# constantinpape/torch-em

Measured on AMD Instinct MI355X. Metric: voxels/sec fwd+bwd, UNet3d 1x128^3 bs=2, higher is better.
Workload: dtype f32-class (forward convs on normalised activations: fp32 operands split into 2 fp16 terms = 22 mantissa bits, lo plane scaled by 2^12 with its own fp32 accumulator, 3 fp16 MFMAs per product; other forward convs 3 bf16 terms / 6 MFMAs; data-gradient convs 2 bf16 terms / 3 MFMAs (16-bit products); WEI

## Files before the change

torch_em_amd/csrc/capi.hip:

```cpp
#include "tem_common.h"
#include "conv_internal.h"
#include "tem_act.h"
#include <stdarg.h>
#include <string.h>

static thread_local char g_err[512] = "";

thread_local TemCallSt tem_call_st = {0, 0};
thread_local TemCallCs tem_call_cs = {0, 0};

void tem_set_error(const char* fmt, ...) {
    va_list ap;
    va_start(ap, fmt);
    vsnprintf(g_err, sizeof(g_err), fmt, ap);
    va_end(ap);
}

extern "C" const char* tem_last_error(void) { return g_err; }

struct TemOption {
    const char* name;
    long long def;
};
static const TemOption g_opt_table[TEM_OPT_COUNT] = {
    {"wgrad_zs", 3},
    {"wgrad_zs_persist", 1},
    {"wgrad_sums", 1},
    {"wgrad_sums_min_mb", 128},
    {"fwd_persistent", -1},
    {"conv_fwd_variant", -1},
    {"conv1x1_stream", 1},
    {"fwd_ksplit_chunks", 0},
    {"wgrad_cus", 256},
    {"upsample_generic", 0},
    {"team_min_units", 0},
    {"zr_splitk", 1},
    {"zr_wide", 1},
    {"zr_tile_blocks", 1},
    {"dice_vox", 1},
    {"upsample2_ch8", 1},
    {"pool_vec8", 2},
    {"fp32_zr", 1},
};
static long long g_opt_val[TEM_OPT_COUNT];
static bool g_opt_set[TEM_OPT_COUNT];

long long tem_option(int id) {
    if (id < 0 || id >= TEM_OPT_COUNT) return 0;
    return __atomic_load_n(&g_opt_set[id], __ATOMIC_RELAXED) ? __atomic_load_n(&g_opt_val[id], __ATOMIC_RELAXED)
                                                            : g_opt_table[id].def;
}
static int opt_find(const char* name) {
    if (!name) return -1;
    for (int i = 0; i < TEM_OPT_COUNT; ++i)
        if (!strcmp(name, g_opt_table[i].name)) return i;
    return -1;
}
extern "C" int tem_set_option(const char* name, int64_t value) {
    const int id = opt_find(name);
    TEM_REQUIRE(id >= 0, "tem_set_option: unknown option '%s'", name ? name : "(null)");
    __atomic_store_n(&g_opt_val[id], (long long)value, __ATOMIC_RELAXED);
    __atomic_store_n(&g_opt_set[id], true, __ATOMIC_RELAXED);
    return TEM_OK;
}
extern "C" int tem_get_option(const char* name, int64_t* value) {
    const int id = opt_find(name);
    TEM_REQUIRE(id >= 0 && value, "tem_get_option: unknown option '%s'", name ? name : "(null)");
    *value = (int64_t)tem_option(id);
    return TEM_OK;
}
extern "C" int tem_version(void) { return 100; }

thread_local TemByproducts* tem_call_bp = nullptr;
unsigned* tem_take_output_amax() {
    TemByproducts* bp = tem_call_bp;
    if (!bp || !bp->out_amax || (bp->delivered & TEM_BP_OUT_AMAX)) return nullptr;
    bp->delivered |= TEM_BP_OUT_AMAX;
    return bp->out_amax;
}
bool tem_bp_wants(unsigned bit) {
    const TemByproducts* bp = tem_call_bp;
    if (!bp || (bp->delivered & bit)) return false;
    return bit == TEM_BP_NORM_COEF ? bp->coef != nullptr : bit == TEM_BP_NORM_SUMS ? bp->sums_part != nullptr : bp->out_amax != nullptr;
}
void tem_bp_delivered(unsigned bit) {
    if (tem_call_bp) tem_call_bp->delivered |= bit;
}

extern "C" int tem_device_cus(void) {
    int dev = 0;
    if (hipGetDevice(&dev) != hipSuccess) return TEM_ELAUNCH;
    hipDeviceProp_t prop;
    if (hipGetDeviceProperties(&prop, dev) != hipSuccess) return TEM_ELAUNCH;
    return prop.multiProcessorCount;
}
// ... 157 lines not shown
```

torch_em_amd/csrc/conv_zr.hip:

```cpp
#include "tem_common.h"
#include "conv_internal.h"
#include "conv_split.h"
#include "tem_act.h"
#include <type_traits>

#ifndef TEM_ZR_PRIO
#define TEM_ZR_PRIO 1
#endif
#ifndef TEM_ZR_STAGE_PRIO
#define TEM_ZR_STAGE_PRIO 0
#endif
#ifndef TEM_ZR_R0
#define TEM_ZR_R0 2
#endif
#ifndef TEM_ZR_R0_16
#define TEM_ZR_R0_16 2
#endif
#ifndef TEM_ZR_R0_16S
#define TEM_ZR_R0_16S 2
#endif
#ifndef TEM_ZR_AD
#define TEM_ZR_AD 2
#endif
#ifndef TEM_ZR_ST_AUX
#define TEM_ZR_ST_AUX 2
#endif
#ifndef TEM_ZR_ST_AUX_KS
#define TEM_ZR_ST_AUX_KS 2
#endif
#ifndef TEM_ZR_X32_SCHED
#define TEM_ZR_X32_SCHED 1
#endif
#ifndef TEM_ZR_X32_R0_M0
#define TEM_ZR_X32_R0_M0 6
#define TEM_ZR_X32_R0_M1 4
#define TEM_ZR_X32_R0_M2 6
#define TEM_ZR_X32_R0_M3 5
#endif
#ifndef TEM_ZR_X32_GAP
#define TEM_ZR_X32_GAP 0
#endif
#ifndef TEM_ZR_ABL
#define TEM_ZR_ABL 0
#endif

typedef float floatx4z __attribute__((ext_vector_type(4)));
typedef float float2v __attribute__((ext_vector_type(2)));
typedef unsigned int u32x4z __attribute__((ext_vector_type(4)));

__device__ __forceinline__ __amdgpu_buffer_rsrc_t zr_rsrc(const void* base) {
    return __builtin_amdgcn_make_buffer_rsrc(const_cast<void*>(base), 0, 0x7fffffff, 0x00020000);
}
__device__ __forceinline__ float4 zr_load4(__amdgpu_buffer_rsrc_t r, unsigned voff, unsigned soff) {
    const u32x4z v = __builtin_amdgcn_raw_buffer_load_b128(r, voff, soff, 0);
    const floatx4z f = __builtin_bit_cast(floatx4z, v);
    return make_float4(f.x, f.y, f.z, f.w);
}
__device__ __forceinline__ uint4 zr_load4u(__amdgpu_buffer_rsrc_t r, unsigned voff, unsigned soff) {
    const u32x4z v = __builtin_amdgcn_raw_buffer_load_b128(r, voff, soff, 0);
    return make_uint4(v.x, v.y, v.z, v.w);
}
template <int AUX>
__device__ __forceinline__ void zr_store4(__amdgpu_buffer_rsrc_t r, unsigned voff, unsigned soff, float a, float b, float c, float d) {
    const u32x4z v = {__builtin_bit_cast(unsigned, a), __builtin_bit_cast(unsigned, b), __builtin_bit_cast(unsigned, c),
                      __builtin_bit_cast(unsigned, d)};
    __builtin_amdgcn_raw_buffer_store_b128(v, r, voff + soff, 0, AUX);
}

__device__ __forceinline__ uint2 zr_load2u(__amdgpu_buffer_rsrc_t r, unsigned voff, unsigned soff) {
    typedef unsigned int u32x2z __attribute__((ext_vector_type(2)));
    const u32x2z v = __builtin_amdgcn_raw_buffer_load_b64(r, voff, soff, 0);
    return make_uint2(v.x, v.y);
}
template <int AUX>
__device__ __forceinline__ void zr_store2u(__amdgpu_buffer_rsrc_t r, unsigned voff, unsigned soff, unsigned a, unsigned b) {
    typedef unsigned int u32x2z __attribute__((ext_vector_type(2)));
    const u32x2z v = {a, b};
    __builtin_amdgcn_raw_buffer_store_b64(v, r, voff + soff, 0, AUX);
}
template <bool F16>
__device__ __forceinline__ unsigned zr_norm2(unsigned h, float s0, float t0, float s1, float t1) {
    if constexpr (F16) {
        unsigned q;
        asm("v_fma_mixlo_f16 %0, %1, %2, %3 op_sel_hi:[1,0,0]" : "=v"(q) : "v"(h), "v"(s0), "v"(t0));
        asm("v_fma_mixhi_f16 %0, %1, %2, %3 op_sel:[1,0,0] op_sel_hi:[1,0,0]" : "+v"(q) : "v"(h), "v"(s1), "v"(t1));
        return q;
    } else {
        const float a = __builtin_bit_cast(float, h << 16), b = __builtin_bit_cast(float, h & 0xffff0000u);
        return pk_bf16(fmaf(a, s0, t0), fmaf(b, s1, t1));
    }
}

template <int M>
__device__ __forceinline__ float zr_swz(float v) {
    return __builtin_bit_cast(float, __builtin_amdgcn_ds_swizzle(__builtin_bit_cast(int, v), (M << 10) | 0x1f));
}

__device__ __forceinline__ float zr_xor16_sum(float r) {
    float a = r, b = r;
    asm volatile("s_nop 1\n\tv_permlane16_swap_b32 %0, %1" : "+v"(a), "+v"(b));
    return a + b;
}
__device__ __forceinline__ float zr_xor32_sum(float r) {
    float a = r, b = r;
    asm volatile("s_nop 1\n\tv_permlane32_swap_b32 %0, %1" : "+v"(a), "+v"(b));
    return a + b;
}

template <int CTRL>
__device__ __forceinline__ float zr_dpp(float v) {
    return __builtin_bit_cast(float, __builtin_amdgcn_update_dpp(0, __builtin_bit_cast(int, v), CTRL, 0xf, 0xf, true));
}

__device__ __forceinline__ unsigned zr_mix_lo(unsigned h, float g0, float g1) {
    unsigned q;
    const float c = -F16_LO_SCALE;
    asm("v_fma_mixlo_f16 %0, %1, %2, %3 op_sel_hi:[1,0,0]" : "=v"(q) : "v"(h), "s"(c), "v"(g0));
    asm("v_fma_mixhi_f16 %0, %1, %2, %3 op_sel:[1,0,0] op_sel_hi:[1,0,0]" : "+v"(q) : "v"(h), "s"(c), "v"(g1));
    return q;
}

#ifdef TEM_ZR_TRACE
#ifndef TEM_ZR_TRACE_BLOCK
#define TEM_ZR_TRACE_BLOCK 0
#endif
__device__ unsigned long long tem_zr_trace_buf[2][64][12];
#define ZR_STAMP(i)                                                                           \
    do {                                                                                      \
        if (blockIdx.x == TEM_ZR_TRACE_BLOCK && tw == 0 && lane == 0 && s < 64)               \
            tem_zr_trace_buf[team][s][i] = __builtin_amdgcn_s_memtime();                      \
    } while (0)
void tem_zr_trace_read(unsigned long long* dst) {
    (void)hipMemcpyFromSymbol(dst, HIP_SYMBOL(tem_zr_trace_buf), sizeof(unsigned long long) * 2 * 64 * 12);
}
#else
#define ZR_STAMP(i) asm volatile("; ZRMARK " #i)
#endif

__device__ __forceinline__ void zr_x32_gap() {
    if constexpr (TEM_ZR_X32_GAP > 0) {
        __builtin_amdgcn_sched_barrier(0);
        constexpr int FULL16 = TEM_ZR_X32_GAP / 16, REST = TEM_ZR_X32_GAP % 16;
#pragma unroll
        for (int i = 0; i < FULL16; ++i) asm volatile("s_nop 15");
        if constexpr (REST > 0) asm volatile("s_nop %0" ::"n"(REST - 1));
        __builtin_amdgcn_sched_barrier(0);
    }
}

__device__ __forceinline__ unsigned zr_ssel_ltu(unsigned a, unsigned b, unsigned t, unsigned f) {
    unsigned r;
    asm volatile("s_cmp_lt_u32 %1, %2\n\ts_cselect_b32 %0, %3, %4" : "=s"(r) : "s"(a), "s"(b), "s"(t), "s"(f) : "scc");
    return r;
}

struct ZrUnit {
    int cot, n, z0, y0, x0, ksl;
};

template <int NS, bool F16, int MODE, bool KSPLIT = false, bool WIDE = false, typename T = float, bool X32 = false, bool XS = false>
__global__ __launch_bounds__(XS ? 256 : 512, XS ? 1 : 2) void k_conv_zr(
    const T* __restrict__ x, int64_t x_ld, const float* __restrict__ scale, const float* __restrict__ shift,
    const uint4* __restrict__ wp, const float* __restrict__ bias, std::conditional_t<KSPLIT, float, T>* __restrict__ y, int64_t y_ld,
    const T* __restrict__ ref, int64_t ref_ld, int N, int D, int H, int W, int Cin, int Cout, int act, int nZ,
    int nY, int nX, float* __restrict__ stat, int nunits, const unsigned* __restrict__ in_amax, int ks, int blk,
    unsigned* __restrict__ out_amax, int64_t x_cs, int64_t y_cs) {
    static_assert(!KSPLIT || MODE == 0, "split-K units write raw partial sums");
    constexpr bool AMAX = MODE == 2 || MODE == 3;
    float amx = 0.f;
    static_assert(!WIDE || NS == 2, "the wide one-term kernel uses the two LDS planes of the two-term layout");
    static_assert(!X32 || (NS == 2 && !F16 && !WIDE && sizeof(T) == 4), "exact fp32: two LDS planes of eight fp32 channels, fp32 tensors");
    static_assert(!XS || X32, "the one-team workgroup exists for the exact-fp32 arithmetic only");
    constexpr bool T16 = sizeof(T) == 2;
    using TOut = std::conditional_t<KSPLIT, float, T>;
    constexpr bool Y16 = sizeof(TOut) == 2;
    constexpr int XB = (int)sizeof(T), YB = (int)sizeof(TOut);
    static_assert(!T16 || WIDE, "16-bit storage: 32 input channels per phase");
    constexpr int CK = WIDE ? 2 * BCK : BCK;
    constexpr int TZ = 4, TY = 16, TX = 8;
    constexpr int HZ = TZ + 2, HY = TY + 2, HX = TX + 2;
    constexpr int HV = HZ * HY * HX;
    constexpr int PLB = HV * 32;
    constexpr int NIT = HZ * 3;
    constexpr int LPV = (WIDE && !T16) ? 8 : 4;
    constexpr int SPP = (WIDE && !T16) ? 6 : 3;
    constexpr int CPL = T16 ? 8 : 4;
    constexpr int RP = NIT / SPP;
    constexpr int R0 = X32 ? (MODE == 0 ? TEM_ZR_X32_R0_M0 : MODE == 1 ? TEM_ZR_X32_R0_M1 : MODE == 2 ? TEM_ZR_X32_R0_M2 : TEM_ZR_X32_R0_M3)
                       : (WIDE && !T16) ? ((MODE == 1 || MODE == 3) ? 1 : 2)
                       : T16 ? ((MODE == 1 || MODE == 3) ? TEM_ZR_R0_16S : TEM_ZR_R0_16)
                             : (TEM_ZR_R0 < HZ ? TEM_ZR_R0 : HZ);
    constexpr int FR = NS * 64;
    constexpr bool SC = F16 && NS == 2 && !WIDE;
    constexpr int ZSTEP = HY * HX * 32;
    static_assert(HY % 2 == 0, "the record-half swizzle (row parity) is the same in every halo plane");
    extern __shared__ __attribute__((aligned(16))) unsigned char zr_lds[];

    if (SC) __builtin_amdgcn_s_setreg(1 | (23 << 6) | (0 << 11), 1);
    const int tid = threadIdx.x, lane = tid & 63;
    const int wv = __builtin_amdgcn_readfirstlane(tid >> 6);
    const int team = wv >> 2, tw = wv & 3, tl = tid & 255;
    const int kh = lane >> 5, v = lane & 31;
    const int vu = (int)((0x73261540u >> (4 * (v >> 2))) & 7u) * 4 + (v & 3);
    const int py = vu >> 3, px = vu & 7;
    unsigned char* lds = zr_lds + team * (NS * PLB);

    const int G = (XS ? 1 : 2) * gridDim.x;
    const int slot = XS ? tem_xcd_remap(blockIdx.x, gridDim.x) : tem_xcd_remap(blockIdx.x, gridDim.x) * 2 + team;
    const int ncot = Cout >> 5;
    const int nch_all = Cin / CK;
    const int nch = KSPLIT ? nch_all / ks : nch_all;
    const int my_units = slot < nunits ? (nunits - slot + G - 1) / G : 0;
    const int P = ((nunits + G - 1) / G) * nch;

    auto decode = [&](int ui) {
        int u = slot + ui * G;
        ZrUnit t;
        t.ksl = 0;
        if (KSPLIT) { t.ksl = u % ks; u /= ks; }
// ... 198 lines not shown
                if ((u & 1) == 0) col_addr(u >> 1);
#pragma unroll
                for (int hz = 0; hz < HZ; ++hz) xr[u & 1][hz] = *reinterpret_cast<const uint4*>(tcur + a0 + hz * ZSTEP + (u & 1) * PLB);
            };
            r_read(0);
#pragma unroll
            for (int u = 0; u < 18; ++u) {
                const int g = u >> 1, p = u & 1;
                if (u + PFD < NSL) stage_load(u + PFD);
                if (u + 1 < 18) r_read(u + 1);
                if (g + 1 < 9 && !(TEM_ZR_ABL & 4)) {
                    const int gn = g + 1;
#pragma unroll
                    for (int tz = (p ? 2 : 0); tz < (p ? 3 : 2); ++tz)
#pragma unroll
                        for (int pp = 0; pp < 2; ++pp)
                            wq[gn & 1][tz][pp] = zr_load4u(rw, woff_lane, wsoff + (unsigned)((tz * 9 + gn) * ts + pp * 64) * 16u);
                }
                if (u >= 15) {
                    const int tz = u - 15;
#pragma unroll
                    for (int pp = 0; pp < 2; ++pp) wqn[tz][pp] = zr_load4u(rw, woff_lane, wsoff_n + (unsigned)((tz * 9) * ts + pp * 64) * 16u);
                }
                stage_conv(u, tnxt);
#pragma unroll
                for (int c = 0; c < 4; ++c)
#pragma unroll
                    for (int tz = 0; tz < 3; ++tz)
#pragma unroll
                        for (int z = 0; z < TZ; ++z)
                            acc[z] = __builtin_amdgcn_mfma_f32_32x32x2f32(comp(wq[g & 1][tz][p], c), comp(xr[u & 1][z + tz], c), acc[z], 0, 0, 0);
                __builtin_amdgcn_sched_barrier(0);
            }
            if (last_chunk) {
                eu = cu;
                bve = bv;
                unsigned yo = yoff_lane, ro = roff_lane;
                asm volatile("" : "+v"(yo), "+v"(ro));
                epilogue_now(yo, ro, ph);
                bv = bias ? bias[tu.cot * 32 + v] : 0.f;
                ++ui;
            }
            cu = tu;
            ci = tc;
#pragma unroll
            for (int tz = 0; tz < 3; ++tz)
#pragma unroll
                for (int p = 0; p < 2; ++p) wq[0][tz][p] = wqn[tz][p];
            __syncthreads();
        }
        if (AMAX && out_amax) tem_amax_commit(out_amax, amx);
        return;
    }
    if (team) __syncthreads();
    for (int s = 0; s <= P; ++s) {
        const bool do_stage = ui < my_units;
        uint4 wq[2][3][NS];
        {
            ZR_STAMP(0);
            if (TEM_ZR_STAGE_PRIO) __builtin_amdgcn_s_setprio(TEM_ZR_STAGE_PRIO);
#pragma unroll
            for (int j = 0; j < SPP; ++j) asm volatile("" : "+v"(lwj[j]), "+v"(poff[j]));
            unsigned yoff_l = yoff_lane, roff_l = roff_lane;
            asm volatile("" : "+v"(yoff_l), "+v"(roff_l));
            float4 tmp[NIT];
            unsigned inb[2] = {0xffffffffu, 0xffffffffu};
            float4 sc4 = make_float4(1.f, 1.f, 1.f, 1.f), sf4 = make_float4(0.f, 0.f, 0.f, 0.f);
            float4 sc5 = sc4, sf5 = sf4;
            bool interior = true;
            __amdgpu_buffer_rsrc_t rx = zr_rsrc(x);
            auto load_norm = [&]() {
                if (scale) {
                    sc4 = *reinterpret_cast<const float4*>(scale + (int64_t)cu.n * Cin + (cu.ksl * nch + ci) * CK + c4 * CPL);
                    sf4 = *reinterpret_cast<const float4*>(shift + (int64_t)cu.n * Cin + (cu.ksl * nch + ci) * CK + c4 * CPL);
                    if (T16) {
                        sc5 = *reinterpret_cast<const float4*>(scale + (int64_t)cu.n * Cin + (cu.ksl * nch + ci) * CK + c4 * CPL + 4);
                        sf5 = *reinterpret_cast<const float4*>(shift + (int64_t)cu.n * Cin + (cu.ksl * nch + ci) * CK + c4 * CPL + 4);
                    }
                } else if (in_amax) {
                    sc4 = make_float4(psc, psc, psc, psc);
                }
            };
            if (do_stage) {
                if constexpr (!X32) load_norm();
                const int64_t xch = (T16 && x_cs) ? (int64_t)(cu.ksl * nch + ci) * x_cs : (int64_t)((cu.ksl * nch + ci) * CK);
                const T* xb = x + ((((int64_t)cu.n * D + (cu.z0 - 1)) * H + (cu.y0 - 1)) * W + (cu.x0 - 1)) * x_ld + xch;
                rx = zr_rsrc((TEM_ZR_ABL & 64) ? x + xch : xb);
                interior = (cu.z0 >= 1) & (cu.z0 + HZ - 1 <= D) & (cu.y0 >= 1) & (cu.y0 + HY - 1 <= H) & (cu.x0 >= 1) &
                           (cu.x0 + HX - 1 <= W);
                if (TEM_ZR_ABL & 32) interior = true;
                if constexpr (X32) {
#pragma unroll
                    for (int hz = 0; hz < R0; ++hz) {
                        const unsigned so = zr_ssel_ltu((unsigned)(cu.z0 - 1 + hz), (unsigned)D, (unsigned)hz * plane_b, plane_b);
#pragma unroll
                        for (int j = 0; j < SPP; ++j) {
                            if (TEM_ZR_ABL & 1) tmp[hz * SPP + j] = make_float4(0.5f + hz, 0.25f, -1.f, 2.f);
                            else tmp[hz * SPP + j] = zr_load4(rx, pvo[X32 ? j : 0], so);
                        }
                    }
                    load_norm();
                }
            }
            unsigned yx = (1u << SPP) - 1u;
            if constexpr (X32) {
                if (do_stage) {
                    yx = yxu;
                    if (!interior) {
                        inb[0] = inb[1] = 0;
#pragma unroll
                        for (int hz = 0; hz < HZ; ++hz) {
                            const bool zok = (unsigned)(cu.z0 - 1 + hz) < (unsigned)D;
#pragma unroll
                            for (int j = 0; j < SPP; ++j)
                                inb[hz / 3] |= (zok & ((yx >> j) & 1u)) ? (1u << ((hz % 3) * SPP + j)) : 0u;
                        }
                    }
                }
            } else
            if (do_stage && !interior) {
                int tl_ = tl;
                asm volatile("" : "+v"(tl_));
                yx = 0;
#pragma unroll
                for (int j = 0; j < SPP; ++j) {
                    const int q = min((tl_ + 256 * j) / LPV, HY * HX - 1);
                    const unsigned gy = (unsigned)(cu.y0 - 1 + q / HX), gx = (unsigned)(cu.x0 - 1 + q % HX);
                    yx |= ((gy < (unsigned)H) & (gx < (unsigned)W)) ? (1u << j) : 0u;
                }
            }
            auto issue_loads = [&](auto interior_tag, auto lo_tag, auto hi_tag) {
                constexpr bool INTERIOR = decltype(interior_tag)::value;
                constexpr int LO = decltype(lo_tag)::value, HI = decltype(hi_tag)::value;
                if (INTERIOR) {
#pragma unroll
                    for (int hz = LO; hz < HI; ++hz)
#pragma unroll
                        for (int j = 0; j < SPP; ++j) {
                            if (TEM_ZR_ABL & 1) tmp[(hz % RP) * SPP + j] = make_float4(0.5f + hz, 0.25f, -1.f, 2.f);
                            else tmp[(hz % RP) * SPP + j] = zr_load4(rx, poff[j], (unsigned)hz * plane_b);
                        }
                } else {
                    if (LO == 0) inb[0] = inb[1] = 0;
#pragma unroll
                    for (int hz = LO; hz < HI; ++hz) {
                        const bool zok = (unsigned)(cu.z0 - 1 + hz) < (unsigned)D;
#pragma unroll
                        for (int j = 0; j < SPP; ++j) {
                            const bool ok = zok & ((yx >> j) & 1u);
                            inb[hz / 3] |= ok ? (1u << ((hz % 3) * SPP + j)) : 0u;
                            tmp[(hz % RP) * SPP + j] = zr_load4(rx, (ok ? poff[j] : ctr_off) + (ok ? (unsigned)hz * plane_b : plane_b), 0);
                        }
                    }
                }
            };
            if (do_stage && !X32) {
                if (interior) issue_loads(std::true_type{}, std::integral_constant<int, 0>{}, std::integral_constant<int, R0>{});
                else issue_loads(std::false_type{}, std::integral_constant<int, 0>{}, std::integral_constant<int, R0>{});
            }
            ZR_STAMP(1);
            if (!X32 && epi_pending) {
#include "conv_zr_epilogue.inc"
                epi_pending = false;
                ZR_STAMP(11);
            }
            ZR_STAMP(6);
            if (do_stage) {
                auto convert = [&](auto interior_tag, auto hz_tag) {
                    constexpr bool INTERIOR = decltype(interior_tag)::value;
                    constexpr int hz = decltype(hz_tag)::value;
#pragma unroll
                    for (int j = 0; j < SPP; ++j) {
                        const int it = (hz % RP) * SPP + j;
                        if constexpr (T16) {
                            if (j < SPP - 1 || slot2) {
                                u32x4z raw = __builtin_bit_cast(u32x4z, floatx4z{tmp[it].x, tmp[it].y, tmp[it].z, tmp[it].w});
                                if (scale) {
                                    raw.x = zr_norm2<F16>(raw.x, sc4.x, sf4.x, sc4.y, sf4.y);
                                    raw.y = zr_norm2<F16>(raw.y, sc4.z, sf4.z, sc4.w, sf4.w);
                                    raw.z = zr_norm2<F16>(raw.z, sc5.x, sf5.x, sc5.y, sf5.y);
                                    raw.w = zr_norm2<F16>(raw.w, sc5.z, sf5.z, sc5.w, sf5.w);
                                }
                                if (!INTERIOR) {
                                    const bool ok = ((inb[hz / 3] >> ((hz % 3) * SPP + j)) & 1u) != 0;
                                    raw.x = ok ? raw.x : 0u; raw.y = ok ? raw.y : 0u; raw.z = ok ? raw.z : 0u; raw.w = ok ? raw.w : 0u;
                                }
                                if (!(TEM_ZR_ABL & 8) || raw.x == 0x12345678u)
                                    *reinterpret_cast<uint4*>(lds + lwj[j] + hz * ZSTEP) = make_uint4(raw.x, raw.y, raw.z, raw.w);
                            }
                        } else
                        if (j < SPP - 1 || slot2) {
                            float m = 1.f;
                            if (!INTERIOR) m = ((inb[hz / 3] >> ((hz % 3) * SPP + j)) & 1u) ? 1.f : 0.f;
                            float e[4] = {fmaf(tmp[it].x, sc4.x, sf4.x), fmaf(tmp[it].y, sc4.y, sf4.y),
                                          fmaf(tmp[it].z, sc4.z, sf4.z), fmaf(tmp[it].w, sc4.w, sf4.w)};
                            if (!INTERIOR) {
#pragma unroll
                                for (int c = 0; c < 4; ++c) e[c] *= m;
                            }
                            unsigned char* dstp = lds + lwj[j] + hz * ZSTEP;
                            if constexpr (X32) {
                                if (!(TEM_ZR_ABL & 8) || e[0] == 12345.678f) *reinterpret_cast<float4*>(dstp) = make_float4(e[0], e[1], e[2], e[3]);
                            } else
                            if (SC) {
                                const half2_t hh0 = {(_Float16)e[0], (_Float16)e[1]}, hh1 = {(_Float16)e[2], (_Float16)e[3]};
                                unsigned u0 = __builtin_bit_cast(unsigned, hh0), u1 = __builtin_bit_cast(unsigned, hh1);
                                if (!(TEM_ZR_ABL & 8) || u0 == 0x12345678u) *reinterpret_cast<uint2*>(dstp) = make_uint2(u0, u1);
                                const float g[4] = {e[0] * F16_LO_SCALE, e[1] * F16_LO_SCALE, e[2] * F16_LO_SCALE, e[3] * F16_LO_SCALE};
                                const unsigned q0 = zr_mix_lo(u0, g[0], g[1]), q1 = zr_mix_lo(u1, g[2], g[3]);
                                if (!(TEM_ZR_ABL & 8) || u0 == 0x12345678u) *reinterpret_cast<uint2*>(dstp + PLB) = make_uint2(q0, q1);
                            } else if (WIDE) {
#pragma unroll
                                for (int c = 0; c < 4; ++c) asm volatile("" : "+v"(e[c]));
                                const unsigned h0 = pk16<F16>(e[0], e[1]), h1 = pk16<F16>(e[2], e[3]);
                                if (!(TEM_ZR_ABL & 8) || h0 == 0x12345678u) *reinterpret_cast<uint2*>(dstp) = make_uint2(h0, h1);
                            } else {
                                if (F16 && NS == 1) {
#pragma unroll
                                    for (int c = 0; c < 4; ++c) asm volatile("" : "+v"(e[c]));
                                }
#pragma unroll
                                for (int p = 0; p < NS; ++p) {
                                    const unsigned h0 = pk16<F16>(e[0], e[1]), h1 = pk16<F16>(e[2], e[3]);
                                    if (!(TEM_ZR_ABL & 8) || h0 == 0x12345678u)
                                        *reinterpret_cast<uint2*>(dstp + p * PLB) = make_uint2(h0, h1);
                                    if (p + 1 < NS) {
                                        e[0] -= lo16<F16>(h0);
                                        e[1] -= hi16<F16>(h0);
                                        e[2] -= lo16<F16>(h1);
                                        e[3] -= hi16<F16>(h1);
                                    }
                                }
                            }
                        }
                    }
                };
                auto stage_planes = [&](auto interior_tag) {
#define ZR_PLANE(HZI)                                                                                              \
    do {                                                                                                           \
        if ((HZI) + R0 < HZ)                                                                                       \
            issue_loads(interior_tag, std::integral_constant<int, ((HZI) + R0 < HZ ? (HZI) + R0 : 0)>{},           \
                        std::integral_constant<int, ((HZI) + R0 < HZ ? (HZI) + R0 + 1 : 0)>{});                    \
        convert(interior_tag, std::integral_constant<int, (HZI)>{});                                               \
    } while (0)
                    ZR_PLANE(0); ZR_PLANE(1); ZR_PLANE(2); ZR_PLANE(3); ZR_PLANE(4); ZR_PLANE(5);
#undef ZR_PLANE
                };
                if (interior) stage_planes(std::true_type{});
                else stage_planes(std::false_type{});
                ZR_STAMP(7);
                wsoff = (unsigned)((cu.cot * 27 * nch_all + cu.ksl * nch + ci) * FR) * 16u;
#pragma unroll
                for (int tz = 0; tz < 3; ++tz)
#pragma unroll
                    for (int p = 0; p < NS; ++p)
                        wq[0][tz][p] = zr_load4u(rw, woff_lane, wsoff + (unsigned)((tz * 9) * tapstride + p * 64) * 16u);
            }
            ZR_STAMP(2);
            if (TEM_ZR_STAGE_PRIO) __builtin_amdgcn_s_setprio(0);
        }
        __syncthreads();
        {
            ZR_STAMP(3);
            if (do_stage) {
                int ts = tapstride;
                asm volatile("" : "+s"(ts));
                if (TEM_ZR_PRIO) __builtin_amdgcn_s_setprio(TEM_ZR_PRIO);
                constexpr int NSTEP = 9 * HZ;
                constexpr int AD = TEM_ZR_AD;
                uint4 af[AD + 1][NS];
                unsigned a0 = 0u;
                const unsigned hsel = (unsigned)((py & 1) ^ kh) << 4;
                int hvb_ = hvb;
                asm volatile("" : "+v"(hvb_));
                auto col_addr = [&](int g) {
                    const int hvv = hvb_ + (g / 3) * HX + (g % 3);
                    a0 = (unsigned)hvv * 32u + (((g / 3) & 1) ? hsel ^ 16u : hsel);
                };
                auto a_read = [&](int st) {
                    const int hz = st % HZ;
#pragma unroll
                    for (int p = 0; p < NS; ++p)
                        af[st % (AD + 1)][p] = *reinterpret_cast<const uint4*>(lds + a0 + hz * ZSTEP + p * PLB);
                };
                if constexpr (X32 && TEM_ZR_X32_SCHED == 1) {
                    uint4 xr[2][HZ];
                    auto r_read = [&](int u) {
                        if ((u & 1) == 0) col_addr(u >> 1);
#pragma unroll
                        for (int hz = 0; hz < HZ; ++hz)
                            xr[u & 1][hz] = *reinterpret_cast<const uint4*>(lds + a0 + hz * ZSTEP + (u & 1) * PLB);
                    };
                    auto comp = [](const uint4& q, int c) {
                        return __builtin_bit_cast(float, c == 0 ? q.x : (c == 1 ? q.y : (c == 2 ? q.z : q.w)));
                    };
                    r_read(0);
#pragma unroll
                    for (int u = 0; u < 18; ++u) {
                        const int g = u >> 1, p = u & 1;
                        if (u + 1 < 18) r_read(u + 1);
                        if (g + 1 < 9 && !(TEM_ZR_ABL & 4)) {
                            const int gn = g + 1;
// ... 168 lines not shown
    if (D < 4 || Cin % 16 || Cout % 32) return g;
    if (tem_call_st.x && (Cin % 32 || !(nsplit == 5 || nsplit == 7))) return g;
    if ((int64_t)H * W * 8 * 4 * max_ld >= (1ll << 31)) return g;
    static int ncu = 0;
    if (!ncu) {
        ncu = tem_device_cus();
        if (ncu <= 0) ncu = 256;
    }
    g.nZ = (D + 3) / 4;
    g.nY = (H + 15) / 16;
    g.nX = (W + 7) / 8;
    g.nunits = (int64_t)N * g.nZ * g.nY * g.nX * (Cout / 32);
    if (g.nunits >= (1ll << 31)) return g;
    const long long minu = tem_option(TEM_OPT_TEAM_MIN_UNITS);
    if (g.nunits < (opt == 2 ? 1 : (minu > 0 ? minu : 2ll * ncu))) return g;
    g.ok = 1;
    return g;
}

int64_t tem_conv_zr_stat_blocks(int N, int D, int H, int W, int Cin, int Cout, int kd, int kh, int kw, int nsplit, int64_t max_ld) {
    const ZrGeom g = zr_geometry(N, D, H, W, Cin, Cout, kd, kh, kw, nsplit, max_ld);
    if (!g.ok) return -1;
    return (int64_t)g.nZ * g.nY * g.nX * 4;
}

static int zr_tile_blocks(const ZrGeom& g) {
    if (!tem_option(TEM_OPT_ZR_TILE_BLOCKS)) return 0;
    auto lg = [](int n) { return n % 4 == 0 ? 2 : (n % 2 == 0 ? 1 : 0); };
    return lg(g.nX) | (lg(g.nY) << 4) | (lg(g.nZ) << 8);
}

template <int NS, bool F16, int MODE, bool KSPLIT = false, bool WIDE = false, typename T = float, bool X32 = false, bool XS = false>
static void zr_launch(const ZrGeom& g, const float* x_, int64_t x_ld, const float* scale, const float* shift, const float* wp,
                      const float* bias, float* y_, int64_t y_ld, const float* ref_, int64_t ref_ld, int N, int D, int H, int W,
                      int Cin, int Cout, int act, float* stat, const unsigned* in_amax, hipStream_t s, int ks = 1) {
    constexpr size_t ldsb = (size_t)2 * NS * 1080 * 32 + 4 * 32 * 144;
    static_assert(ldsb <= 160 * 1024, "LDS budget");
    const T* x = reinterpret_cast<const T*>(x_);
    const T* ref = reinterpret_cast<const T*>(ref_);
    auto* y = reinterpret_cast<std::conditional_t<KSPLIT, float, T>*>(y_);
    auto kern = &k_conv_zr<NS, F16, MODE, KSPLIT, WIDE, T, X32, XS>;
    static bool attr = false;
    if (!attr) {
        (void)hipFuncSetAttribute(reinterpret_cast<const void*>(kern), hipFuncAttributeMaxDynamicSharedMemorySize, (int)ldsb);
        attr = true;
    }
    static int ncu = 0;
    if (!ncu) {
        ncu = tem_device_cus();
        if (ncu <= 0) ncu = 256;
    }
    int64_t grid = XS ? g.nunits : (g.nunits + 1) / 2;
    if (grid > ncu) grid = ncu;
    unsigned* const out_amax = (MODE == 2 || MODE == 3) ? tem_take_output_amax() : nullptr;
    hipLaunchKernelGGL(kern, dim3((unsigned)grid), dim3(XS ? 256 : 512), ldsb, s, x, x_ld, scale, shift, reinterpret_cast<const uint4*>(wp),
                       bias, y, y_ld, ref, ref_ld, N, D, H, W, Cin, Cout, act, g.nZ, g.nY, g.nX, stat, (int)g.nunits, in_amax, ks,
                       zr_tile_blocks(g), out_amax, (int64_t)(sizeof(T) == 2 ? tem_call_cs.x : 0), (int64_t)(sizeof(T) == 2 && !KSPLIT ? tem_call_cs.y : 0));
}

#ifndef TEM_ZR_KS_FILL
#define TEM_ZR_KS_FILL 4
#endif
int tem_conv_zr_splitk_ks(int N, int D, int H, int W, int Cin, int Cout, int kd, int kh, int kw, int nsplit) {
    const long long opt = tem_option(TEM_OPT_CONV_FWD_VARIANT);
    if (opt == 0 || opt == 1 || !tem_option(TEM_OPT_ZR_SPLITK)) return 0;
    if (!(nsplit == 2 || nsplit == 4 || nsplit == 5 || nsplit == 7 || (nsplit == 1 && tem_option(TEM_OPT_FP32_ZR) && !tem_call_st.x))) return 0;
    if (!(kd == 3 && kh == 3 && kw == 3) || D < 4 || Cin % 16 || Cout % 32) return 0;
    const bool t16 = tem_call_st.x != 0;
    if (t16 && (Cin % 32 || !(nsplit == 5 || nsplit == 7))) return 0;
    if (zr_geometry(N, D, H, W, Cin, Cout, kd, kh, kw, nsplit, 1).ok) return 0;
    if (tem_conv_pp_tiles(N, D, H, W, Cin, Cout, kd, kh, kw, nsplit, 1)) return 0;
    static int ncu = 0;
    if (!ncu) {
        ncu = tem_device_cus();
        if (ncu <= 0) ncu = 256;
    }
    const int nZ = (D + 3) / 4, nY = (H + 15) / 16, nX = (W + 7) / 8;
    if ((int64_t)D * H * W * 10 < (int64_t)nZ * 4 * nY * 16 * nX * 8 * TEM_ZR_KS_FILL) return 0;
    const int64_t units = (int64_t)N * nZ * nY * nX * (Cout / 32);
    const int nch = Cin / 16;
    for (int d = 2; d <= nch / 2; ++d)
        if (nch % d == 0 && units * d >= 2ll * ncu && !(t16 && (nch / d) % 2)) return d;
    return 0;
}

int tem_conv_fwd_zr_splitk(const float* x, int64_t x_ld, const float* scale, const float* shift, const float* wp,
                           const float* bias, float* y, int64_t y_ld, const float* ref, int64_t ref_ld, void* ws,
                           int64_t ws_bytes, int N, int D, int H, int W, int Cin, int Cout, int kd, int kh, int kw, int act,
                           int nsplit, float* stat, hipStream_t s) {
    const int ks = ws ? tem_conv_zr_splitk_ks(N, D, H, W, Cin, Cout, kd, kh, kw, nsplit) : 0;
    if (!ks) return 0;
    if (stat && !tem_splitk_stat_blocks((int64_t)D * H * W, Cout)) return 0;
    if ((int64_t)H * W * 8 * 4 * (x_ld > Cout ? x_ld : Cout) >= (1ll << 31)) return 0;
    if ((y_ld % 4) || ((uintptr_t)y % 16) || (ref && ((ref_ld % 4) || ((uintptr_t)ref % 16))) || (bias && ((uintptr_t)bias % 16)))
        return 0;
    const int64_t NV = (int64_t)N * D * H * W;
    if (ws_bytes < (int64_t)ks * NV * Cout * 4) return 0;
    ZrGeom g = {};
    g.nZ = (D + 3) / 4;
    g.nY = (H + 15) / 16;
    g.nX = (W + 7) / 8;
    g.nunits = (int64_t)N * g.nZ * g.nY * g.nX * (Cout / 32) * ks;
    g.ok = 1;
    float* part = (float*)ws;
#define ZRKS(NS, F16, WIDE)                                                                                            \
    zr_launch<NS, F16, 0, true, WIDE>(g, x, x_ld, scale, shift, wp, nullptr, part, Cout, nullptr, 0, N, D, H, W, Cin, Cout,  \
                                      TEM_ACT_NONE, nullptr, nullptr, s, ks)
// ... 14 lines not shown
    else if (nsplit == 7 && wide) ZRKS(2, false, true);
    else if (nsplit == 5) ZRKS(1, true, false);
    else if (nsplit == 7) ZRKS(1, false, false);
    else if (nsplit == 4) ZRKS(2, true, false);
    else ZRKS(2, false, false);
#undef ZRKS
    TemDgradSumsReq rq = {nullptr, 0, nullptr, nullptr, 0, nullptr, 0};
    if (!stat && tem_bp_wants(TEM_BP_NORM_SUMS)) {
        const TemByproducts* bp = tem_call_bp;
        rq = TemDgradSumsReq{bp->sums_x, bp->sums_x_ld, bp->sums_mean, bp->sums_rstd, bp->sums_G, bp->sums_part, bp->sums_nblk};
    }
    if (stat)
        tem_splitk_epilogue_stats(part, ks, N, (int64_t)D * H * W, Cout, bias, act, ref, ref_ld, y, y_ld, stat, s);
    else if (rq.part && rq.x && rq.mean && rq.rstd && rq.nblk == tem_splitk_stat_blocks((int64_t)D * H * W, Cout) && rq.G > 0 &&
             Cout % rq.G == 0 && rq.x_ld % 4 == 0 && ((uintptr_t)rq.x % 16 == 0)) {
        tem_bp_delivered(TEM_BP_NORM_SUMS);
        tem_splitk_epilogue_bwd_sums(part, ks, N, (int64_t)D * H * W, Cout, bias, act, ref, ref_ld, y, y_ld, rq, s);
    } else
        tem_splitk_epilogue(part, ks, NV, Cout, bias, act, ref, ref_ld, y, y_ld, s);
    return 1;
}

int64_t tem_conv_zr_splitk_stat_blocks(int N, int D, int H, int W, int Cin, int Cout, int kd, int kh, int kw, int nsplit) {
    if (!tem_conv_zr_splitk_ks(N, D, H, W, Cin, Cout, kd, kh, kw, nsplit)) return -1;
    const int64_t nb = tem_splitk_stat_blocks((int64_t)D * H * W, Cout);
    return nb > 0 ? nb : -1;
}

thread_local const unsigned* tem_zr_in_amax = nullptr;
thread_local const float* tem_zr_ref_coef = nullptr;

int tem_conv_fwd_zr(const float* x, int64_t x_ld, const float* scale, const float* shift, const float* wp, const float* bias,
                    float* y, int64_t y_ld, const float* ref, int64_t ref_ld, int N, int D, int H, int W, int Cin, int Cout,
                    int kd, int kh, int kw, int act, int nsplit, float* stat, hipStream_t s) {
    int64_t max_ld = x_ld > y_ld ? x_ld : y_ld;
    if (ref && ref_ld > max_ld) max_ld = ref_ld;
    const ZrGeom g = zr_geometry(N, D, H, W, Cin, Cout, kd, kh, kw, nsplit, max_ld);
    const bool strided = tem_call_cs.x != 0 || tem_call_cs.y != 0;
    if (strided && (!g.ok || !tem_call_st.x || ref || (tem_call_cs.x && Cin % 32) || (tem_call_cs.x % 8) || (tem_call_cs.y % 8))) {
        tem_set_error("tem_conv3d_fwd_ex: chunk strides (x_cs / y_cs) need 16-bit tensors on the z-reuse kernel (tem_conv3d_fwd_kernel() "
                      "== 3), no ref, strides %% 8 == 0");
        return -1;
    }
    if (!g.ok) return 0;
    if ((y_ld % 4) || ((uintptr_t)y % 16) || (ref && ((ref_ld % 4) || ((uintptr_t)ref % 16))) || (stat && ref) ||
        (bias && ((uintptr_t)bias % 16)) || act == TEM_ACT_SIGMOID) {
        if (stat || strided) {
            tem_set_error("tem_conv3d_fwd_stats / _ex: statistics (or chunk strides) were sized for the z-reuse kernel but this launch "
                          "cannot take it (y / ref / bias need 16-byte alignment and ld %% 4 == 0, no ref, no sigmoid)");
            return -1;
        }
        return 0;
    }
#define ZRGO(NS, F16, WIDE)                                                                                                   \
    do {                                                                                                                      \
        if (stat)                                                                                                             \
            zr_launch<NS, F16, 1, false, WIDE>(g, x, x_ld, scale, shift, wp, bias, y, y_ld, ref, ref_ld, N, D, H, W, Cin, Cout, act, stat, in_amax, s); \
        else if (ref && rcoef)                                                                                                \
            zr_launch<NS, F16, 3, false, WIDE>(g, x, x_ld, scale, shift, wp, bias, y, y_ld, ref, ref_ld, N, D, H, W, Cin, Cout, act,        \
                                  const_cast<float*>(rcoef), in_amax, s);                                                     \
        else if (ref)                                                                                                         \
            zr_launch<NS, F16, 2, false, WIDE>(g, x, x_ld, scale, shift, wp, bias, y, y_ld, ref, ref_ld, N, D, H, W, Cin, Cout, act, stat, in_amax, s); \
        else                                                                                                                  \
            zr_launch<NS, F16, 0, false, WIDE>(g, x, x_ld, scale, shift, wp, bias, y, y_ld, ref, ref_ld, N, D, H, W, Cin, Cout, act, stat, in_amax, s); \
    } while (0)
    const float* rcoef = tem_zr_ref_coef;
    if (rcoef) {
        if (!ref || stat || ((uintptr_t)rcoef % 16)) {
            tem_set_error("tem_conv3d_fwd_refnorm: needs ref, no statistics, 16-byte aligned coefficients");
            return -1;
        }
        tem_zr_ref_coef = nullptr;
    }
    const unsigned* in_amax = tem_zr_in_amax;
    if (in_amax) {
        if (nsplit != 4 || bias || scale || stat) {
            tem_set_error("tem_conv3d_fwd_gscaled: fp16 two-term layout, no bias / norm / statistics");
            return -1;
        }
        tem_zr_in_amax = nullptr;
    }
    const bool wide = (nsplit == 5 || nsplit == 7) && Cin % 32 == 0 && tem_option(TEM_OPT_ZR_WIDE);
#define ZRGO16(F16, T)                                                                                                        \
    do {                                                                                                                      \
        if (stat)                                                                                                             \
            zr_launch<2, F16, 1, false, true, T>(g, x, x_ld, scale, shift, wp, bias, y, y_ld, ref, ref_ld, N, D, H, W, Cin, Cout, act, stat, in_amax, s); \
        else if (ref && rcoef)                                                                                                \
            zr_launch<2, F16, 3, false, true, T>(g, x, x_ld, scale, shift, wp, bias, y, y_ld, ref, ref_ld, N, D, H, W, Cin, Cout, act,        \
                                  const_cast<float*>(rcoef), in_amax, s);                                                     \
        else if (ref)                                                                                                         \
            zr_launch<2, F16, 2, false, true, T>(g, x, x_ld, scale, shift, wp, bias, y, y_ld, ref, ref_ld, N, D, H, W, Cin, Cout, act, stat, in_amax, s); \
        else                                                                                                                  \
            zr_launch<2, F16, 0, false, true, T>(g, x, x_ld, scale, shift, wp, bias, y, y_ld, ref, ref_ld, N, D, H, W, Cin, Cout, act, stat, in_amax, s); \
    } while (0)
#define ZRGO32S()                                                                                                               \
    do {                                                                                                                      \
        if (stat)                                                                                                             \
            zr_launch<2, false, 1, false, false, float, true, true>(g, x, x_ld, scale, shift, wp, bias, y, y_ld, ref, ref_ld, N, D, H, W, Cin, Cout, act, stat, in_amax, s); \
        else if (ref && rcoef)                                                                                                \
            zr_launch<2, false, 3, false, false, float, true, true>(g, x, x_ld, scale, shift, wp, bias, y, y_ld, ref, ref_ld, N, D, H, W, Cin, Cout, act,        \
                                  const_cast<float*>(rcoef), in_amax, s);                                                     \
        else if (ref)                                                                                                         \
            zr_launch<2, false, 2, false, false, float, true, true>(g, x, x_ld, scale, shift, wp, bias, y, y_ld, ref, ref_ld, N, D, H, W, Cin, Cout, act, stat, in_amax, s); \
        else                                                                                                                  \
            zr_launch<2, false, 0, false, false, float, true, true>(g, x, x_ld, scale, shift, wp, bias, y, y_ld, ref, ref_ld, N, D, H, W, Cin, Cout, act, stat, in_amax, s); \
    } while (0)
#define ZRGO32()                                                                                                                \
    do {                                                                                                                      \
        if (stat)                                                                                                             \
            zr_launch<2, false, 1, false, false, float, true>(g, x, x_ld, scale, shift, wp, bias, y, y_ld, ref, ref_ld, N, D, H, W, Cin, Cout, act, stat, in_amax, s); \
        else if (ref && rcoef)                                                                                                \
            zr_launch<2, false, 3, false, false, float, true>(g, x, x_ld, scale, shift, wp, bias, y, y_ld, ref, ref_ld, N, D, H, W, Cin, Cout, act,        \
                                  const_cast<float*>(rcoef), in_amax, s);                                                     \
        else if (ref)                                                                                                         \
            zr_launch<2, false, 2, false, false, float, true>(g, x, x_ld, scale, shift, wp, bias, y, y_ld, ref, ref_ld, N, D, H, W, Cin, Cout, act, stat, in_amax, s); \
        else                                                                                                                  \
            zr_launch<2, false, 0, false, false, float, true>(g, x, x_ld, scale, shift, wp, bias, y, y_ld, ref, ref_ld, N, D, H, W, Cin, Cout, act, stat, in_amax, s); \
    } while (0)
    if (tem_call_st.x == 1) ZRGO16(true, tem_f16);
    else if (tem_call_st.x == 2) ZRGO16(false, tem_bf16);
    else
#undef ZRGO16
    if (nsplit == 1 && tem_option(TEM_OPT_FP32_ZR) == 2) ZRGO32S();
    else if (nsplit == 1) ZRGO32();
    else if (nsplit == 5 && wide) ZRGO(2, true, true);
    else if (nsplit == 7 && wide) ZRGO(2, false, true);
    else if (nsplit == 5) ZRGO(1, true, false);
    else if (nsplit == 7) ZRGO(1, false, false);
    else if (nsplit == 4) ZRGO(2, true, false);
    else ZRGO(2, false, false);
#undef ZRGO
#undef ZRGO32
#undef ZRGO32S
    return 1;
}
```

torch_em_amd/csrc/tem_common.h:

```cpp
#pragma once
#include <hip/hip_runtime.h>
#include <stdint.h>
#include <stdio.h>
#include "../../include/tem_hip.h"

void tem_set_error(const char* fmt, ...);

enum {
    TEM_OPT_WGRAD_ZS = 0,
    TEM_OPT_WGRAD_ZS_PERSIST,
    TEM_OPT_WGRAD_SUMS,
    TEM_OPT_WGRAD_SUMS_MIN_MB,
    TEM_OPT_FWD_PERSISTENT,
    TEM_OPT_CONV_FWD_VARIANT,
    TEM_OPT_CONV1X1_STREAM,
    TEM_OPT_FWD_KSPLIT_CHUNKS,
    TEM_OPT_WGRAD_CUS,
    TEM_OPT_UPSAMPLE_GENERIC,
    TEM_OPT_TEAM_MIN_UNITS,
    TEM_OPT_ZR_SPLITK,
    TEM_OPT_ZR_WIDE,
    TEM_OPT_ZR_TILE_BLOCKS,
    TEM_OPT_DICE_VOX,
    TEM_OPT_UPSAMPLE2_CH8,
    TEM_OPT_POOL_VEC8,
    TEM_OPT_FP32_ZR,
    TEM_OPT_COUNT
};
long long tem_option(int id);

#define TEM_REQUIRE(cond, ...)                 \
    do {                                       \
        if (!(cond)) {                         \
            tem_set_error(__VA_ARGS__);        \
            return TEM_EINVAL;                 \
        }                                      \
    } while (0)

#define TEM_CHECK_LAUNCH(name)                                                   \
    do {                                                                         \
        hipError_t e__ = hipGetLastError();                                      \
        if (e__ != hipSuccess) {                                                 \
            tem_set_error("%s: launch failed: %s", name, hipGetErrorString(e__)); \
            return TEM_ELAUNCH;                                                  \
        }                                                                        \
    } while (0)

static inline int64_t tem_cdiv(int64_t a, int64_t b) { return (a + b - 1) / b; }
static inline int64_t tem_align_up(int64_t a, int64_t b) { return tem_cdiv(a, b) * b; }

static inline int tem_grid_1d(int64_t work_items, int block, int max_blocks = 256 * 8) {
    int64_t g = tem_cdiv(work_items, block);
    if (g > max_blocks) g = max_blocks;
    if (g < 1) g = 1;
    return (int)g;
}

#define TEM_WAVE 64

extern thread_local TemByproducts* tem_call_bp;
struct TemBpScope {
    TemByproducts* prev;
    explicit TemBpScope(TemByproducts* bp) : prev(tem_call_bp) {
        tem_call_bp = bp;
        if (bp) bp->delivered = 0;
    }
    ~TemBpScope() { tem_call_bp = prev; }
};
bool tem_bp_wants(unsigned bit);
void tem_bp_delivered(unsigned bit);
unsigned* tem_take_output_amax();
__device__ __forceinline__ float tem_amax4(float m, float a, float b, float c, float d) {
    return __builtin_fmaxf(__builtin_fmaxf(m, __builtin_fmaxf(__builtin_fabsf(a), __builtin_fabsf(b))),
                           __builtin_fmaxf(__builtin_fabsf(c), __builtin_fabsf(d)));
}
__device__ __forceinline__ void tem_amax_commit(unsigned* amax, float m) {
    unsigned u = __builtin_bit_cast(unsigned, m);
#pragma unroll
    for (int o = 32; o > 0; o >>= 1) u = max(u, (unsigned)__shfl_xor((int)u, o, 64));
// ... 22 lines not shown
```

Measured before the change: 282.5 million.

## Load paired channel chunks together in zr conv staging to fill wider cache lines

Adds a paired-lines mode to the zr 3D conv kernel, used for the bf16x3 fp32-storage path with no stats or residual. When a stage handles an even channel chunk, it also loads the next chunk's 32 bytes from the same voxel lines into registers. The following stage then converts from those held registers and issues no global loads. The aim is better cache-line use and fewer load round trips, at the cost of many more live registers (a hold array of NIT vectors) and a reordered epilogue, which may reduce occupancy or cause spills.

```diff
diff --git a/torch_em_amd/csrc/capi.hip b/torch_em_amd/csrc/capi.hip
--- a/torch_em_amd/csrc/capi.hip
+++ b/torch_em_amd/csrc/capi.hip
@@ -41,6 +41,7 @@
     {"upsample2_ch8", 1},
     {"pool_vec8", 2},
     {"fp32_zr", 1},
+    {"zr_lines", 1},
 };
 static long long g_opt_val[TEM_OPT_COUNT];
 static bool g_opt_set[TEM_OPT_COUNT];
diff --git a/torch_em_amd/csrc/conv_zr.hip b/torch_em_amd/csrc/conv_zr.hip
--- a/torch_em_amd/csrc/conv_zr.hip
+++ b/torch_em_amd/csrc/conv_zr.hip
@@ -55,6 +55,9 @@
     const u32x4z v = __builtin_amdgcn_raw_buffer_load_b128(r, voff, soff, 0);
     const floatx4z f = __builtin_bit_cast(floatx4z, v);
     return make_float4(f.x, f.y, f.z, f.w);
+}
+__device__ __forceinline__ floatx4z zr_load4x(__amdgpu_buffer_rsrc_t r, unsigned voff, unsigned soff) {
+    return __builtin_bit_cast(floatx4z, __builtin_amdgcn_raw_buffer_load_b128(r, voff, soff, 0));
 }
 __device__ __forceinline__ uint4 zr_load4u(__amdgpu_buffer_rsrc_t r, unsigned voff, unsigned soff) {
     const u32x4z v = __builtin_amdgcn_raw_buffer_load_b128(r, voff, soff, 0);
@@ -158,13 +161,16 @@
     int cot, n, z0, y0, x0, ksl;
 };
 
-template <int NS, bool F16, int MODE, bool KSPLIT = false, bool WIDE = false, typename T = float, bool X32 = false, bool XS = false>
+template <int NS, bool F16, int MODEP, bool KSPLIT = false, bool WIDE = false, typename T = float, bool X32 = false, bool XS = false>
 __global__ __launch_bounds__(XS ? 256 : 512, XS ? 1 : 2) void k_conv_zr(
     const T* __restrict__ x, int64_t x_ld, const float* __restrict__ scale, const float* __restrict__ shift,
     const uint4* __restrict__ wp, const float* __restrict__ bias, std::conditional_t<KSPLIT, float, T>* __restrict__ y, int64_t y_ld,
     const T* __restrict__ ref, int64_t ref_ld, int N, int D, int H, int W, int Cin, int Cout, int act, int nZ,
     int nY, int nX, float* __restrict__ stat, int nunits, const unsigned* __restrict__ in_amax, int ks, int blk,
     unsigned* __restrict__ out_amax, int64_t x_cs, int64_t y_cs) {
+    constexpr int MODE = MODEP & 3;
+    constexpr bool LN = (MODEP & 4) != 0;
+    static_assert(!LN || (NS == 2 && !F16 && !KSPLIT && !WIDE && sizeof(T) == 4 && !X32), "paired lines: bf16x3 with fp32 storage");
     static_assert(!KSPLIT || MODE == 0, "split-K units write raw partial sums");
     constexpr bool AMAX = MODE == 2 || MODE == 3;
     float amx = 0.f;
@@ -469,9 +475,12 @@
         if (AMAX && out_amax) tem_amax_commit(out_amax, amx);
         return;
     }
+    floatx4z hold[LN ? NIT : 1];
     if (team) __syncthreads();
     for (int s = 0; s <= P; ++s) {
         const bool do_stage = ui < my_units;
+        const bool lfirst = LN && do_stage && !(ci & 1) && ci + 1 < nch;
+        const bool lsecond = LN && do_stage && (ci & 1);
         uint4 wq[2][3][NS];
         {
             ZR_STAMP(0);
@@ -485,7 +494,7 @@
             float4 sc4 = make_float4(1.f, 1.f, 1.f, 1.f), sf4 = make_float4(0.f, 0.f, 0.f, 0.f);
             float4 sc5 = sc4, sf5 = sf4;
             bool interior = true;
-            __amdgpu_buffer_rsrc_t rx = zr_rsrc(x);
+            __amdgpu_buffer_rsrc_t rx = zr_rsrc(x), rx2 = rx;
             auto load_norm = [&]() {
                 if (scale) {
                     sc4 = *reinterpret_cast<const float4*>(scale + (int64_t)cu.n * Cin + (cu.ksl * nch + ci) * CK + c4 * CPL);
@@ -503,6 +512,7 @@
                 const int64_t xch = (T16 && x_cs) ? (int64_t)(cu.ksl * nch + ci) * x_cs : (int64_t)((cu.ksl * nch + ci) * CK);
                 const T* xb = x + ((((int64_t)cu.n * D + (cu.z0 - 1)) * H + (cu.y0 - 1)) * W + (cu.x0 - 1)) * x_ld + xch;
                 rx = zr_rsrc((TEM_ZR_ABL & 64) ? x + xch : xb);
+                if (LN) rx2 = zr_rsrc(((TEM_ZR_ABL & 64) ? x + xch : xb) + CK);
                 interior = (cu.z0 >= 1) & (cu.z0 + HZ - 1 <= D) & (cu.y0 >= 1) & (cu.y0 + HY - 1 <= H) & (cu.x0 >= 1) &
                            (cu.x0 + HX - 1 <= W);
                 if (TEM_ZR_ABL & 32) interior = true;
@@ -546,17 +556,24 @@
                     yx |= ((gy < (unsigned)H) & (gx < (unsigned)W)) ? (1u << j) : 0u;
                 }
             }
-            auto issue_loads = [&](auto interior_tag, auto lo_tag, auto hi_tag) {
+            auto issue_loads = [&](auto interior_tag, auto lo_tag, auto hi_tag, auto lm_tag) {
                 constexpr bool INTERIOR = decltype(interior_tag)::value;
                 constexpr int LO = decltype(lo_tag)::value, HI = decltype(hi_tag)::value;
+                constexpr int LM = decltype(lm_tag)::value;
                 if (INTERIOR) {
-#pragma unroll
-                    for (int hz = LO; hz < HI; ++hz)
-#pragma unroll
-                        for (int j = 0; j < SPP; ++j) {
-                            if (TEM_ZR_ABL & 1) tmp[(hz % RP) * SPP + j] = make_float4(0.5f + hz, 0.25f, -1.f, 2.f);
-                            else tmp[(hz % RP) * SPP + j] = zr_load4(rx, poff[j], (unsigned)hz * plane_b);
-                        }
+                    if constexpr (LM != 2) {
+#pragma unroll
+                        for (int hz = LO; hz < HI; ++hz)
+#pragma unroll
+                            for (int j = 0; j < SPP; ++j) {
+                                if (TEM_ZR_ABL & 1) tmp[(hz % RP) * SPP + j] = make_float4(0.5f + hz, 0.25f, -1.f, 2.f);
+                                else tmp[(hz % RP) * SPP + j] = zr_load4(rx, poff[j], (unsigned)hz * plane_b);
+                                if constexpr (LM == 1) {
+                                    if (TEM_ZR_ABL & 1) hold[LN ? hz * SPP + j : 0] = floatx4z{0.5f + hz, 0.25f, -1.f, 2.f};
+                                    else hold[LN ? hz * SPP + j : 0] = zr_load4x(rx2, poff[j], (unsigned)hz * plane_b);
+                                }
+                            }
+                    }
                 } else {
                     if (LO == 0) inb[0] = inb[1] = 0;
 #pragma unroll
@@ -566,26 +583,46 @@
                         for (int j = 0; j < SPP; ++j) {
                             const bool ok = zok & ((yx >> j) & 1u);
                             inb[hz / 3] |= ok ? (1u << ((hz % 3) * SPP + j)) : 0u;
-                            tmp[(hz % RP) * SPP + j] = zr_load4(rx, (ok ? poff[j] : ctr_off) + (ok ? (unsigned)hz * plane_b : plane_b), 0);
+                            if constexpr (LM == 0) {
+                                tmp[(hz % RP) * SPP + j] = zr_load4(rx, (ok ? poff[j] : ctr_off) + (ok ? (unsigned)hz * plane_b : plane_b), 0);
+                            } else if constexpr (LM == 1) {
+                                const unsigned o = (ok ? poff[j] : ctr_off) + (ok ? (unsigned)hz * plane_b : plane_b);
+                                tmp[(hz % RP) * SPP + j] = zr_load4(rx, o, 0);
+                                hold[LN ? hz * SPP + j : 0] = zr_load4x(rx2, o, 0);
+                            }
                         }
                     }
                 }
             };
+            auto with_lm = [&](auto f) {
+                if (lfirst) f(std::integral_constant<int, 1>{});
+                else if (lsecond) f(std::integral_constant<int, 2>{});
+                else f(std::integral_constant<int, 0>{});
+            };
             if (do_stage && !X32) {
-                if (interior) issue_loads(std::true_type{}, std::integral_constant<int, 0>{}, std::integral_constant<int, R0>{});
-                else issue_loads(std::false_type{}, std::integral_constant<int, 0>{}, std::integral_constant<int, R0>{});
+                if constexpr (LN) {
+                    with_lm([&](auto lm) {
+                        constexpr int R0S = decltype(lm)::value == 1 ? (R0 + 1) / 2 : R0;
+                        if (interior) issue_loads(std::true_type{}, std::integral_constant<int, 0>{}, std::integral_constant<int, R0S>{}, lm);
+                        else issue_loads(std::false_type{}, std::integral_constant<int, 0>{}, std::integral_constant<int, R0S>{}, lm);
+                    });
+                } else {
+                    if (interior) issue_loads(std::true_type{}, std::integral_constant<int, 0>{}, std::integral_constant<int, R0>{}, std::integral_constant<int, 0>{});
+                    else issue_loads(std::false_type{}, std::integral_constant<int, 0>{}, std::integral_constant<int, R0>{}, std::integral_constant<int, 0>{});
+                }
             }
             ZR_STAMP(1);
-            if (!X32 && epi_pending) {
+            if (!X32 && epi_pending && !lsecond) {
 #include "conv_zr_epilogue.inc"
                 epi_pending = false;
                 ZR_STAMP(11);
             }
             ZR_STAMP(6);
             if (do_stage) {
-                auto convert = [&](auto interior_tag, auto hz_tag) {
+                auto convert = [&](auto interior_tag, auto hz_tag, auto lm_tag) {
                     constexpr bool INTERIOR = decltype(interior_tag)::value;
                     constexpr int hz = decltype(hz_tag)::value;
+                    constexpr int LM = decltype(lm_tag)::value;
 #pragma unroll
                     for (int j = 0; j < SPP; ++j) {
                         const int it = (hz % RP) * SPP + j;
@@ -609,8 +646,10 @@
                         if (j < SPP - 1 || slot2) {
                             float m = 1.f;
                             if (!INTERIOR) m = ((inb[hz / 3] >> ((hz % 3) * SPP + j)) & 1u) ? 1.f : 0.f;
-                            float e[4] = {fmaf(tmp[it].x, sc4.x, sf4.x), fmaf(tmp[it].y, sc4.y, sf4.y),
-                                          fmaf(tmp[it].z, sc4.z, sf4.z), fmaf(tmp[it].w, sc4.w, sf4.w)};
+                            const float4 t4 = LM == 2 ? make_float4(hold[LN ? hz * SPP + j : 0].x, hold[LN ? hz * SPP + j : 0].y,
+                                                                    hold[LN ? hz * SPP + j : 0].z, hold[LN ? hz * SPP + j : 0].w)
+                                                      : tmp[it];
+                            float e[4] = {fmaf(t4.x, sc4.x, sf4.x), fmaf(t4.y, sc4.y, sf4.y), fmaf(t4.z, sc4.z, sf4.z), fmaf(t4.w, sc4.w, sf4.w)};
                             if (!INTERIOR) {
 #pragma unroll
                                 for (int c = 0; c < 4; ++c) e[c] *= m;
@@ -652,19 +691,27 @@
                         }
                     }
                 };
-                auto stage_planes = [&](auto interior_tag) {
+                auto stage_planes = [&](auto interior_tag, auto lm_tag) {
+                    constexpr int R0S = decltype(lm_tag)::value == 1 ? (R0 + 1) / 2 : R0;
 #define ZR_PLANE(HZI)                                                                                              \
     do {                                                                                                           \
-        if ((HZI) + R0 < HZ)                                                                                       \
-            issue_loads(interior_tag, std::integral_constant<int, ((HZI) + R0 < HZ ? (HZI) + R0 : 0)>{},           \
-                        std::integral_constant<int, ((HZI) + R0 < HZ ? (HZI) + R0 + 1 : 0)>{});                    \
-        convert(interior_tag, std::integral_constant<int, (HZI)>{});                                               \
+        if ((HZI) + R0S < HZ)                                                                                      \
+            issue_loads(interior_tag, std::integral_constant<int, ((HZI) + R0S < HZ ? (HZI) + R0S : 0)>{},         \
+                        std::integral_constant<int, ((HZI) + R0S < HZ ? (HZI) + R0S + 1 : 0)>{}, lm_tag);          \
+        convert(interior_tag, std::integral_constant<int, (HZI)>{}, lm_tag);                                       \
     } while (0)
                     ZR_PLANE(0); ZR_PLANE(1); ZR_PLANE(2); ZR_PLANE(3); ZR_PLANE(4); ZR_PLANE(5);
 #undef ZR_PLANE
                 };
-                if (interior) stage_planes(std::true_type{});
-                else stage_planes(std::false_type{});
+                if constexpr (LN) {
+                    with_lm([&](auto lm) {
+                        if (interior) stage_planes(std::true_type{}, lm);
+                        else stage_planes(std::false_type{}, lm);
+                    });
+                } else {
+                    if (interior) stage_planes(std::true_type{}, std::integral_constant<int, 0>{});
+                    else stage_planes(std::false_type{}, std::integral_constant<int, 0>{});
+                }
                 ZR_STAMP(7);
                 wsoff = (unsigned)((cu.cot * 27 * nch_all + cu.ksl * nch + ci) * FR) * 16u;
 #pragma unroll
@@ -939,7 +986,7 @@
     }
     int64_t grid = XS ? g.nunits : (g.nunits + 1) / 2;
     if (grid > ncu) grid = ncu;
-    unsigned* const out_amax = (MODE == 2 || MODE == 3) ? tem_take_output_amax() : nullptr;
+    unsigned* const out_amax = ((MODE & 3) == 2 || (MODE & 3) == 3) ? tem_take_output_amax() : nullptr;
     hipLaunchKernelGGL(kern, dim3((unsigned)grid), dim3(XS ? 256 : 512), ldsb, s, x, x_ld, scale, shift, reinterpret_cast<const uint4*>(wp),
                        bias, y, y_ld, ref, ref_ld, N, D, H, W, Cin, Cout, act, g.nZ, g.nY, g.nX, stat, (int)g.nunits, in_amax, ks,
                        zr_tile_blocks(g), out_amax, (int64_t)(sizeof(T) == 2 ? tem_call_cs.x : 0), (int64_t)(sizeof(T) == 2 && !KSPLIT ? tem_call_cs.y : 0));
@@ -1060,7 +1107,7 @@
         }
         return 0;
     }
-#define ZRGO(NS, F16, WIDE)                                                                                                   \
+#define ZRGO(NS, F16, WIDE)                                                                                                    \
     do {                                                                                                                      \
         if (stat)                                                                                                             \
             zr_launch<NS, F16, 1, false, WIDE>(g, x, x_ld, scale, shift, wp, bias, y, y_ld, ref, ref_ld, N, D, H, W, Cin, Cout, act, stat, in_amax, s); \
@@ -1136,6 +1183,8 @@
     else if (nsplit == 5) ZRGO(1, true, false);
     else if (nsplit == 7) ZRGO(1, false, false);
     else if (nsplit == 4) ZRGO(2, true, false);
+    else if (!stat && !ref && Cin >= 32 && tem_option(TEM_OPT_ZR_LINES))
+        zr_launch<2, false, 0 | 4>(g, x, x_ld, scale, shift, wp, bias, y, y_ld, ref, ref_ld, N, D, H, W, Cin, Cout, act, stat, in_amax, s);
     else ZRGO(2, false, false);
 #undef ZRGO
 #undef ZRGO32
diff --git a/torch_em_amd/csrc/tem_common.h b/torch_em_amd/csrc/tem_common.h
--- a/torch_em_amd/csrc/tem_common.h
+++ b/torch_em_amd/csrc/tem_common.h
@@ -25,6 +25,7 @@
     TEM_OPT_UPSAMPLE2_CH8,
     TEM_OPT_POOL_VEC8,
     TEM_OPT_FP32_ZR,
+    TEM_OPT_ZR_LINES,
     TEM_OPT_COUNT
 };
 long long tem_option(int id);
```

Measured after the change: 283.0 million (median of 6 runs). No clear change (+0.2%).
